# uce/flink-cooccurrence

Hardware: AMD Instinct MI355X
Metric: item-pair co-occurrences counted/sec (node) at 1/2/4/8 GPUs; achieved HBM GB/s (higher is better)
Workload: dtype u32

## Files before the change

flink-cooccurrence_amd/csrc/cooc_sparse.hip:

```cpp
#include "cooc_sparse.h"
#include <algorithm>
#include <cstdio>
#include <string>

namespace cooc {

namespace {

constexpr int kMaxProbe = 64;
constexpr int kSpU = 4;

template <int kWaves>
__device__ inline uint32_t block_excl_scan(uint32_t x, uint32_t *total, uint32_t *s_wtot) {
  const int lane = threadIdx.x & 63, wave = threadIdx.x >> 6;
  const uint32_t inc = wave_incl_scan(x);
  if (lane == 63) s_wtot[wave] = inc;
  __syncthreads();
  uint32_t pre = 0, tot = 0;
#pragma unroll
  for (int w = 0; w < kWaves; w++) {
    const uint32_t v = s_wtot[w];
    pre += w < wave ? v : 0u;
    tot += v;
  }
  __syncthreads();
  *total = uni(tot);
  return pre + inc - x;
}

struct SpShared {
  uint32_t *R;
  uint32_t *L1;
  uint32_t *L1pre;
  int32_t *gb;
  uint32_t *info;
  uint32_t *vst;
  int32_t *qstart;
};

struct SpStatic {
  uint32_t wtot[kSpWaves];
  uint64_t red[kSpWaves];
  int32_t work;
  uint32_t flag;
  int64_t slab_cur, slab_end, row_begin, row_n, pos, copy_from, copy_n;
  int64_t saved_cur, saved_end;
  uint32_t own;
  uint32_t bstart[kSpMaxTiles + 1];
  uint32_t bcur[kSpMaxTiles];
  uint64_t ovf;
  unsigned long long rsum;
#ifdef COOC_SP_STATS
  unsigned long long st[64];
#endif
};

__device__ inline void sp_hash_insert4(uint32_t *keys, uint32_t *cnts, const uint4 &v, uint32_t hshift, uint32_t hmask,
                                       SpStatic &S_) {
  uint32_t k[4] = {v.x + 1u, v.y + 1u, v.z + 1u, v.w + 1u};
  uint32_t h[4];
#pragma unroll
  for (int i = 0; i < 4; i++) h[i] = (k[i] - 1u) * 0x9E3779B1u >> hshift;
#ifdef COOC_SP_STATS
  if (threadIdx.x == 0) S_.st[24] += (k[0] != 0u) + (k[1] != 0u) + (k[2] != 0u) + (k[3] != 0u);
#endif
  for (int p = 0; p < kMaxProbe; p++) {
#ifdef COOC_SP_STATS
    if (threadIdx.x == 0) S_.st[25] += 1;
#endif
    uint32_t cur[4];
#pragma unroll
    for (int i = 0; i < 4; i++) cur[i] = k[i] ? atomicCAS(keys + h[i], 0u, k[i]) : 0u;
    bool left = false;
#pragma unroll
    for (int i = 0; i < 4; i++) {
      if (!k[i]) continue;
      if (cur[i] == 0u || cur[i] == k[i]) {
        atomicAdd(cnts + h[i], 1u);
        k[i] = 0u;
      } else {
        h[i] = (h[i] + 1u) & hmask;
        left = true;
      }
    }
    if (!left) return;
  }
  S_.flag = 1u;
}

constexpr int kWalkDense = 0;
constexpr int kWalkHash = 1;
constexpr int kWalkGather = 2;
struct WalkOp {
  int mode;
  uint32_t hshift, hmask;
  int64_t sbase;
#ifdef COOC_SP_STATS
  bool split;
#endif
};

template <int kOff, int kW>
__device__ inline uint32_t sp_bits(uint32_t w) {
  uint32_t r;
  asm("v_bfe_u32 %0, %1, %2, %3" : "=v"(r) : "v"(w), "n"(kOff), "n"(kW));
  return r;
}

template <class Sh, int kSh>
__device__ inline void sp_dense_add_bit(uint32_t *R, uint32_t w, uint32_t bit) {
  if (Sh::kU16)
    atomicAdd(&R[sp_bits<kSh + 1, kTShift - 1>(w)], bit << (((w >> kSh) & 1u) << 4));
  else
    atomicAdd(&R[sp_bits<kSh, kTShift>(w)], bit);
}

template <class Sh, int kIds, int kMode>
__device__ inline void sp_apply_group(const SpArgs &A, const SpShared &L, SpStatic &S_, const WalkOp &op,
                                      const uint4 &v, uint32_t m) {
  const uint32_t w[4] = {v.x, v.y, v.z, v.w};
  if (kMode == kWalkHash) {
    uint32_t x[kIds];
#pragma unroll
    for (int i = 0; i < 4; i++) {
      if (kIds == 4) {
        x[i] = w[i];
      } else {
        x[2 * i] = w[i] & 0xFFFFu;
        x[2 * i + 1] = w[i] >> 16;
      }
    }
#pragma unroll
    for (int i = 0; i < kIds; i++)
      if (!((m >> i) & 1u)) x[i] = kSink;
#pragma unroll
    for (int h = 0; h < kIds; h += 4)
      sp_hash_insert4(L.R, L.R + Sh::kHashMax, make_uint4(x[h], x[h + 1], x[h + 2], x[h + 3]), op.hshift, op.hmask, S_);
  } else if (kMode == kWalkGather && kIds == 4) {
    uint32_t *scr = reinterpret_cast<uint32_t *>(A.scratch + op.sbase);
#pragma unroll
    for (int i = 0; i < 4; i++) {
      if (!((m >> i) & 1u)) continue;
      const uint32_t t = w[i] >> kTShift;
      const uint32_t slot = atomicAdd(&S_.bcur[t], 1u);
      if (slot < S_.bstart[t + 1] - S_.bstart[t]) scr[S_.bstart[t] + slot] = w[i];
    }
  } else if (kIds == 4) {
#pragma unroll
    for (int i = 0; i < 4; i++) sp_dense_add_bit<Sh, 0>(L.R, w[i], (m >> i) & 1u);
  } else {
#pragma unroll
    for (int i = 0; i < 4; i++) {
      sp_dense_add_bit<Sh, 0>(L.R, w[i], (m >> (2 * i)) & 1u);
      sp_dense_add_bit<Sh, 16>(L.R, w[i], (m >> (2 * i + 1)) & 1u);
    }
  }
// ... 97 lines not shown
      }
#pragma unroll
      for (int k = 0; k < kSpU; k++) v[k] = vn[k];
      m = mn;
    }
  }
  __syncthreads();
  if (kMode == kWalkHash) STAT_ADD(17, STAT_CLOCK() - c_b1);
  return total;
}

template <class Sh>
__device__ inline uint64_t sp_walk(const SpArgs &A, const SpShared &L, SpStatic &S_, int64_t k0, int64_t k1, int t0,
                                   int t1, bool full, bool bucket, const WalkOp &op) {
  uint64_t walked = 0;
  const int tid = threadIdx.x;
  const bool okt = SP_CHECK(A, t0 >= 0 && t1 <= A.T && t0 <= t1);
  const bool has0 = !bucket && (full || t0 == 0);
  const int ta = full ? 1 : max(t0, 1), tz = full ? A.T : t1;
  const bool has1 = bucket || tz > ta;
  if (bucket) {
    k0 = 0;
    k1 = t1 - t0;
  }
  const uint4 *const ar1 = bucket ? A.scratch + op.sbase : A.tarena;
  const int64_t nsrc1 = bucket ? A.scr_cap : A.n_groups;
  const bool rec = !bucket && A.tbc && (full || (t0 == 0 && !has1));
  constexpr uint32_t kNoList = 0xFFFFFFFFu;
  auto list_of = [&](int64_t b) -> uint32_t {
    if (b + tid >= k1 || !okt) return kNoList;
    const uint32_t u = SP_CHECK(A, b + tid < A.n_contrib) ? A.vals[b + tid] & kListMask : 0u;
    return SP_CHECK(A, u < A.n_users) ? u : 0u;
  };
  auto rec_of = [&](uint32_t u) -> int4 { return u != kNoList ? A.tbc[u] : make_int4(0, 0, 0, 0); };
  int4 rn = make_int4(0, 0, 0, 0);
  uint32_t un = kNoList;
  static_assert(Sh::kDb == Sh::kThreads, "a batch: one contribution per thread");
  if (rec && Sh::kAhead) {
    const uint32_t u0 = list_of(k0);
    un = list_of(k0 + Sh::kDb);
    rn = rec_of(u0);
  }
  for (int64_t b0 = k0; b0 < k1; b0 += Sh::kDb) {
    const int nb = int(min<int64_t>(Sh::kDb, k1 - b0));
    uint32_t s0 = 0, e0 = 0, s1 = 0, e1 = 0;
    STAT_ADD(19, op.mode == kWalkHash && !bucket ? 1 : 0);
    if (bucket) {
      if (tid < nb) {
        s1 = S_.bstart[t0 + tid];
        e1 = s1 + S_.bcur[t0 + tid];
      }
    } else if (rec) {
      if (!Sh::kAhead) rn = rec_of(list_of(b0));
      s0 = uint32_t(rn.x);
      e0 = uint32_t(rn.y);
      if (has1) {
        s1 = uint32_t(rn.z);
        e1 = uint32_t(rn.w);
      }
      if (Sh::kAhead) {
        rn = rec_of(un);
        un = list_of(b0 + 2 * Sh::kDb);
      }
    } else if (tid < nb && okt) {
      const uint32_t u = SP_CHECK(A, b0 + tid < A.n_contrib) ? A.vals[b0 + tid] & kListMask : 0u;
      const int32_t *tbu = A.tb + int64_t(SP_CHECK(A, u < A.n_users) ? u : 0u) * (A.T + 2);
      if (has0) {
        s0 = uint32_t(tbu[0]);
        e0 = uint32_t(tbu[A.T + 1]);
      }
      if (has1) {
        s1 = uint32_t(tbu[ta]);
        e1 = uint32_t(tbu[tz]);
      }
    }
    const unsigned long long c_w0 = STAT_CLOCK();
    if (has0) {
      if (op.mode == kWalkHash)
        walked += sp_walk_batch<Sh, 8, kWalkHash>(A, L, S_, A.tarena0, A.n_groups0, nb, s0, e0, op);
      else
        walked += sp_walk_batch<Sh, 8, kWalkDense>(A, L, S_, A.tarena0, A.n_groups0, nb, s0, e0, op);
    }
    const unsigned long long c_w1 = STAT_CLOCK();
    if (has1) {
      if (op.mode == kWalkHash)
        walked += sp_walk_batch<Sh, 4, kWalkHash>(A, L, S_, ar1, nsrc1, nb, s1, e1, op);
      else if (op.mode == kWalkGather)
        walked += sp_walk_batch<Sh, 4, kWalkGather>(A, L, S_, ar1, nsrc1, nb, s1, e1, op);
      else
        walked += sp_walk_batch<Sh, 4, kWalkDense>(A, L, S_, ar1, nsrc1, nb, s1, e1, op);
    }
#ifdef COOC_SP_STATS
    if (op.split) {
      STAT_ADD(56, c_w1 - c_w0);
      STAT_ADD(57, STAT_CLOCK() - c_w1);
    }
#endif
    if (uni(S_.flag)) break;
  }
  return walked;
}

__device__ inline void sp_global_sync() {
  __builtin_amdgcn_s_waitcnt(0);
  __syncthreads();
  __builtin_amdgcn_fence(__ATOMIC_ACQUIRE, "agent");
}

template <class Sh>
__device__ inline int64_t sp_reserve(const SpArgs &A, SpStatic &S_, int64_t n) {
  const int tid = threadIdx.x;
  if (tid == 0) {
    S_.copy_n = 0;
    if (S_.slab_cur + n > S_.slab_end) {
      const int64_t need = S_.row_n + n;
      const int64_t take = max(A.slab, need + need / 2);
      int64_t b = int64_t(atomicAdd(A.bump, (unsigned long long)take));
      if (b + take > A.cap) {
        atomicOr(reinterpret_cast<unsigned long long *>(&A.tot->err), 4ull);
        S_.pos = -1;
      } else {
        S_.copy_from = S_.row_begin;
        S_.copy_n = S_.row_n;
        S_.row_begin = b;
        S_.slab_cur = b + S_.row_n;
        S_.slab_end = b + take;
        S_.pos = S_.slab_cur;
        S_.slab_cur += n;
      }
    } else {
      S_.pos = S_.slab_cur;
      S_.slab_cur += n;
    }
    if (S_.pos >= 0) S_.row_n += n;
  }
  __syncthreads();
  const int64_t cn = uni(S_.copy_n);
  if (cn > 0) {
    sp_global_sync();
    const int64_t from = S_.copy_from, to = S_.row_begin;
    for (int64_t i = tid; i < cn; i += Sh::kThreads) {
      if (SP_CHECK(A, to + i < A.cap && from + i < A.cap && from >= 0)) {
        A.col_out[to + i] = A.col_out[from + i];
        A.cnt_out[to + i] = A.cnt_out[from + i];
      }
    }
  }
  return uni(S_.pos);
}

template <class Sh>
__device__ inline void sp_dense_compact(const SpArgs &A, const SpShared &L, SpStatic &S_, int32_t w, int32_t c0,
                                        uint64_t &rsum, uint32_t *mdst) {
  constexpr int kPer = Sh::kPer, kStep = 64 * kPer, kQ = kPer / 4;
  const int tid = threadIdx.x, lane = tid & 63, wave = tid >> 6;
  const unsigned long long c_d0 = STAT_CLOCK();
  uint32_t *row = L.R;
  if (mdst) {
    const int32_t mh = min(w, A.mirror_hi);
    for (int32_t i = tid; i < mh; i += Sh::kThreads) {
      const uint32_t v = Sh::kU16 ? (row[i >> 1] >> ((i & 1) << 4)) & 0xFFFFu : row[i];
      if (!v) continue;
      const int32_t sl = A.mslot[i];
      if (sl >= 0) mdst[int64_t(sl) * A.sstride] = v;
    }
  }
  const int32_t per = ((w + Sh::kWaves - 1) / Sh::kWaves + kStep - 1) & ~(kStep - 1);
  const int32_t lo = min(w, wave * per), hi = min(w, lo + per);
  const uint4 *row4 = reinterpret_cast<const uint4 *>(row);
  auto load = [&](int32_t b, uint32_t v[kPer]) {
    if (b < hi) {
      const uint4 q = row4[b / kPer];
      const uint32_t ww[4] = {q.x, q.y, q.z, q.w};
#pragma unroll
      for (int k = 0; k < kPer; k++) {
        const uint32_t x = Sh::kU16 ? (ww[k >> 1] >> (16 * (k & 1))) & 0xFFFFu : ww[k & 3];
        v[k] = b + k < hi ? x : 0u;
      }
    } else {
#pragma unroll
      for (int k = 0; k < kPer; k++) v[k] = 0u;
    }
  };
  uint32_t cnt = 0;
  for (int32_t b0 = lo; b0 < hi; b0 += kStep) {
    uint32_t v[kPer];
    load(b0 + kPer * lane, v);
#pragma unroll
    for (int k = 0; k < kPer; k++) cnt += v[k] != 0u;
  }
  for (int o = 32; o > 0; o >>= 1) cnt += __shfl_xor(cnt, o, 64);
  if (lane == 0) S_.wtot[wave] = cnt;
  __syncthreads();
  STAT_ADD(48, STAT_CLOCK() - c_d0);
  uint32_t off = 0, tot = 0;
#pragma unroll
  for (int wv = 0; wv < Sh::kWaves; wv++) {
    const uint32_t x = S_.wtot[wv];
    off += wv < wave ? x : 0u;
    tot += x;
  }
  const bool map = A.hot_col != nullptr && c0 == 0;
  auto colq = [&](int32_t b, uint4 q[kQ]) {
#pragma unroll
    for (int j = 0; j < kQ; j++)
      q[j] = (map && b < hi) ? *reinterpret_cast<const uint4 *>(A.hot_col + b + 4 * j) : make_uint4(0u, 0u, 0u, 0u);
  };
  uint4 q0[kQ], q1[kQ];
  colq(lo + kPer * lane, q0);
  colq(lo + kStep + kPer * lane, q1);
  const int64_t base = sp_reserve<Sh>(A, S_, tot);
  STAT_ADD(49, STAT_CLOCK() - c_d0);
  const uint64_t lt_mask = (lane == 0) ? 0ull : (~0ull >> (64 - lane));
  for (int32_t b0 = lo; b0 < hi; b0 += kStep) {
    const int32_t b = b0 + kPer * lane;
    uint32_t ids[kPer];
#pragma unroll
    for (int j = 0; j < kQ; j++) {
      ids[4 * j] = q0[j].x;
      ids[4 * j + 1] = q0[j].y;
      ids[4 * j + 2] = q0[j].z;
      ids[4 * j + 3] = q0[j].w;
      q0[j] = q1[j];
    }
    colq(b0 + 2 * kStep + kPer * lane, q1);
    uint32_t v[kPer];
    load(b, v);
    uint32_t c = 0;
#pragma unroll
    for (int k = 0; k < kPer; k++) c += v[k] != 0u;
    const uint64_t m0 = __ballot(c & 1u), m1 = __ballot(c & 2u), m2 = __ballot(c & 4u);
    const uint64_t m3 = kPer > 4 ? __ballot(c & 8u) : 0ull;
    const uint32_t pre = uint32_t(__popcll(m0 & lt_mask)) + 2u * uint32_t(__popcll(m1 & lt_mask)) +
                         4u * uint32_t(__popcll(m2 & lt_mask)) + 8u * uint32_t(__popcll(m3 & lt_mask));
#pragma unroll
    for (int k = 0; k < kPer; k++) rsum += v[k];
    if (c) {
      int64_t pos = base + off + pre;
#pragma unroll
      for (int k = 0; k < kPer; k++) {
        if (!v[k]) continue;
        if (base >= 0) {
          if (SP_CHECK(A, pos >= 0 && pos < A.cap)) {
            A.col_out[pos] = map ? int32_t(ids[k]) : c0 + b + k - (A.hot_col ? kTW : 0);
            A.cnt_out[pos] = v[k];
          }
        }
        pos++;
      }
      reinterpret_cast<uint4 *>(row)[b / kPer] = make_uint4(0u, 0u, 0u, 0u);
    }
    off += uint32_t(__popcll(m0)) + 2u * uint32_t(__popcll(m1)) + 4u * uint32_t(__popcll(m2)) +
           8u * uint32_t(__popcll(m3));
  }
  STAT_ADD(50, STAT_CLOCK() - c_d0);
  __syncthreads();
  STAT_ADD(51, STAT_CLOCK() - c_d0);
}

template <class Sh>
__device__ inline void sp_hash_compact(const SpArgs &A, const SpShared &L, SpStatic &S_, int32_t H, int32_t c0,
                                       int32_t c1, uint64_t &rsum, uint32_t *mdst) {
  const int tid = threadIdx.x;
  const unsigned long long c_h0 = STAT_CLOCK();
  const uint32_t mhi = mdst ? uint32_t(A.mirror_hi) : 0u;
  uint32_t *keys = L.R, *cnts = L.R + Sh::kHashMax;
  const int per = H / Sh::kThreads;
  const int32_t nL1 = (c1 - c0 + 1023) >> 10;
  uint32_t ek[Sh::kHashMax / Sh::kThreads], ec[Sh::kHashMax / Sh::kThreads], er[Sh::kHashMax / Sh::kThreads];
  (void)per;
#pragma unroll
  for (int q = 0; q < Sh::kHashMax / (4 * Sh::kThreads); q++) {
    const int j = 4 * (tid + q * Sh::kThreads);
    uint4 k4 = make_uint4(0u, 0u, 0u, 0u), v4 = k4;
    if (j < H) {
      k4 = *reinterpret_cast<const uint4 *>(keys + j);
      v4 = *reinterpret_cast<const uint4 *>(cnts + j);
      *reinterpret_cast<uint4 *>(keys + j) = make_uint4(0u, 0u, 0u, 0u);
      *reinterpret_cast<uint4 *>(cnts + j) = make_uint4(0u, 0u, 0u, 0u);
    }
    const uint32_t kk[4] = {k4.x, k4.y, k4.z, k4.w}, vv[4] = {v4.x, v4.y, v4.z, v4.w};
#pragma unroll
    for (int u = 0; u < 4; u++) {
      const int i = 4 * q + u;
      ek[i] = ~0u;
      ec[i] = 0u;
      er[i] = 0u;
      if (kk[u] && vv[u]) {
        const uint32_t col = kk[u] - 1u - uint32_t(c0);
        ek[i] = col;
        ec[i] = vv[u];
        rsum += vv[u];
        if (col < mhi) {
          const int32_t sl = A.mslot[col];
          if (sl >= 0) mdst[int64_t(sl) * A.sstride] = vv[u];
        }
        if (Sh::kRank && !A.any_order) atomicOr(&L.L1[col >> 10], 1u << ((col >> 5) & 31u));
      }
    }
  }
  __syncthreads();
  STAT_ADD(46, STAT_CLOCK() - c_h0);
  if (!Sh::kRank || A.any_order) {
    uint32_t cnt = 0;
#pragma unroll
    for (int i = 0; i < Sh::kHashMax / Sh::kThreads; i++) cnt += ek[i] != ~0u;
    uint32_t ne;
    uint32_t q = block_excl_scan<Sh::kWaves>(cnt, &ne, S_.wtot);
    const unsigned long long c_a1 = STAT_CLOCK();
    STAT_ADD(20, c_a1 - c_h0);
    const int64_t base = sp_reserve<Sh>(A, S_, ne);
    const unsigned long long c_a2 = STAT_CLOCK();
    STAT_ADD(21, c_a2 - c_a1);
    if (base >= 0 && ne <= uint32_t(Sh::kWStage)) {
      uint32_t *sc = keys + Sh::kWStage, *sn = cnts + Sh::kWStage;
#pragma unroll
      for (int i = 0; i < Sh::kHashMax / Sh::kThreads; i++) {
        if (ek[i] == ~0u) continue;
        sc[q] = uint32_t(sp_col(A, uint32_t(c0) + ek[i]));
        sn[q] = ec[i];
        q++;
      }
      __syncthreads();
      const uint32_t head = min(ne, uint32_t((4 - (base & 3)) & 3));
      const uint32_t body = (ne - head) >> 2;
      for (uint32_t j = tid; j < head; j += Sh::kThreads) {
        A.col_out[base + j] = int32_t(sc[j]);
        A.cnt_out[base + j] = sn[j];
      }
      int4 *co4 = reinterpret_cast<int4 *>(A.col_out + base + head);
      uint4 *cn4 = reinterpret_cast<uint4 *>(A.cnt_out + base + head);
      for (uint32_t j = tid; j < body; j += Sh::kThreads) {
        const uint32_t r = head + 4 * j;
        co4[j] = make_int4(int32_t(sc[r]), int32_t(sc[r + 1]), int32_t(sc[r + 2]), int32_t(sc[r + 3]));
        cn4[j] = make_uint4(sn[r], sn[r + 1], sn[r + 2], sn[r + 3]);
      }
      for (uint32_t r = head + 4 * body + tid; r < ne; r += Sh::kThreads) {
        A.col_out[base + r] = int32_t(sc[r]);
        A.cnt_out[base + r] = sn[r];
      }
      __syncthreads();
      for (uint32_t r = tid; r < ne; r += Sh::kThreads) {
        sc[r] = 0u;
        sn[r] = 0u;
      }
    } else if (base >= 0) {
#pragma unroll
      for (int i = 0; i < Sh::kHashMax / Sh::kThreads; i++) {
        if (ek[i] == ~0u) continue;
        if (SP_CHECK(A, base + q < A.cap)) {
          A.col_out[base + q] = sp_col(A, uint32_t(c0) + ek[i]);
          A.cnt_out[base + q] = ec[i];
        }
        q++;
      }
    }
    __syncthreads();
    STAT_ADD(22, STAT_CLOCK() - c_a2);
    STAT_ADD(23, ne);
    return;
  }
  if constexpr (Sh::kRank) {
  uint32_t nblk;
  {
    static_assert(Sh::kL1Words % Sh::kThreads == 0, "L1 words per thread");
    constexpr int kW = Sh::kL1Words / Sh::kThreads;
    uint32_t pc[kW], x = 0;
#pragma unroll
    for (int i = 0; i < kW; i++) {
      pc[i] = kW * tid + i < nL1 ? uint32_t(__popc(L.L1[kW * tid + i])) : 0u;
      x += pc[i];
    }
    const uint32_t p = block_excl_scan<Sh::kWaves>(x, &nblk, S_.wtot);
    uint32_t run = p;
#pragma unroll
    for (int i = 0; i < kW; i++) {
      if (kW * tid + i < nL1) L.L1pre[kW * tid + i] = run;
      run += pc[i];
    }
  }
  __syncthreads();
#pragma unroll
  for (int i = 0; i < Sh::kHashMax / Sh::kThreads; i++) {
    if (ek[i] == ~0u) continue;
    const uint32_t col = ek[i], wd = col >> 10, bit = (col >> 5) & 31u;
    const uint32_t r = L.L1pre[wd] + uint32_t(__popc(L.L1[wd] & ((1u << bit) - 1u)));
    er[i] = r;
    atomicOr(&keys[r], 1u << (col & 31u));
  }
  __syncthreads();
  STAT_ADD(47, STAT_CLOCK() - c_h0);
  const uint32_t pb = (nblk + Sh::kThreads - 1) / Sh::kThreads;
  const uint32_t r0 = min(nblk, uint32_t(tid) * pb), r1 = min(nblk, r0 + pb);
  uint32_t local = 0;
  for (uint32_t r = r0; r < r1; r++) local += uint32_t(__popc(keys[r]));
  uint32_t ne;
  uint32_t run = block_excl_scan<Sh::kWaves>(local, &ne, S_.wtot);
  for (uint32_t r = r0; r < r1; r++) {
    cnts[r] = run;
    run += uint32_t(__popc(keys[r]));
  }
  const unsigned long long c_h1 = STAT_CLOCK();
  STAT_ADD(20, c_h1 - c_h0);
  const int64_t base = sp_reserve<Sh>(A, S_, ne);
  const unsigned long long c_h2 = STAT_CLOCK();
  STAT_ADD(21, c_h2 - c_h1);
  if (base >= 0 && ne <= uint32_t(Sh::kWStage)) {
// ... 209 lines not shown
        __syncthreads();
        STAT_ADD(26, STAT_CLOCK() - c_walked);
      } else if (dense) {
        if (tid == 0 && ra >= c0 && ra < c1) {
          const uint32_t o = uint32_t(ra - c0);
          if (Sh::kU16)
            L.R[o >> 1] -= self << ((o & 1u) << 4);
          else
            L.R[o] -= self;
        }
        __syncthreads();
        sp_dense_compact<Sh>(A, L, S_, c1 - c0, c0, rsum, c0 == 0 ? mdst : nullptr);
        STAT_ADD(2, STAT_CLOCK() - c_walked);
      } else {
        if (tid == 0 && ra >= c0 && ra < c1) {
          uint32_t h = (uint32_t(ra) * 0x9E3779B1u) >> op.hshift;
          for (int p = 0; p < H; p++) {
            if (L.R[h] == uint32_t(ra) + 1u) {
              L.R[Sh::kHashMax + h] -= self;
              break;
            }
            h = (h + 1u) & op.hmask;
          }
        }
        __syncthreads();
        sp_hash_compact<Sh>(A, L, S_, H, c0, c1, rsum, c0 == 0 ? mdst : nullptr);
        STAT_ADD(3, STAT_CLOCK() - c_walked);
#ifdef COOC_SP_STATS
        STAT_ADD(30 + 6 * hcls, STAT_CLOCK() - c_walked);
        STAT_ADD(32 + 6 * hcls, uni(S_.row_n));
#endif
        STAT_ADD(14, H);
      }
      t = t1;
      H = 0;
    }
    STAT_ADD(split ? 12 : 11, 1);
    if (deferred) {
      STAT_ADD(8, 1);
      rsum = 0;
      if (tid == 0) {
        A.deferred[atomicAdd(reinterpret_cast<unsigned long long *>(&A.tot->n_deferred), 1ull)] = a;
        if (!S_.own) S_.slab_cur = S_.row_begin;
        S_.row_n = 0;
      }
    }
    if (!split) {
      for (int o = 32; o > 0; o >>= 1) rsum += __shfl_xor(rsum, o, 64);
      if ((tid & 63) == 0 && rsum) atomicAdd(&S_.rsum, (unsigned long long)rsum);
    }
    rsum = 0;
    if (!split && tid == 0) {
      A.row_base[a] = S_.row_n ? S_.row_begin : 0;
      A.row_nnz[a] = int32_t(S_.row_n);
      if (S_.own) {
        S_.slab_cur = S_.saved_cur;
        S_.slab_end = S_.saved_end;
      }
    }
    if (tid == 0) S_.work = next;
    __syncthreads();
    if (!split && !deferred && tid == 0 && S_.rsum != (unsigned long long)rs_expect) {
      atomicOr(reinterpret_cast<unsigned long long *>(&A.tot->err), 2ull);
      A.tot->bad_row = a;
    }
  }
#ifdef COOC_SP_STATS
  if (tid == 0) {
    S_.st[13] = STAT_CLOCK() - t_start;
    for (int k = 0; k < 64; k++) atomicAdd(A.stats + k, S_.st[k]);
  }
#endif
}

constexpr int kFinThreads = 1024, kFinWaves = kFinThreads / 64, kFinU = 4;
__global__ __launch_bounds__(kFinThreads) void k_sp_split_finalize(const int32_t *__restrict__ split_row,
                                                                    const uint32_t *__restrict__ staging, int64_t stride,
                                                                    int32_t M, const int64_t *__restrict__ row_ptr,
                                                                    const int64_t *__restrict__ rowsum,
                                                                    int32_t *__restrict__ col_out,
                                                                    uint32_t *__restrict__ cnt_out,
                                                                    unsigned long long *__restrict__ bump, int64_t cap,
                                                                    int64_t *__restrict__ row_base,
                                                                    int32_t *__restrict__ row_nnz,
                                                                    PlanTotals *__restrict__ tot,
                                                                    const int64_t *__restrict__ spre,
                                                                    const int32_t *__restrict__ hot_col,
                                                                    const int32_t *__restrict__ pos_of) {
  __shared__ uint32_t s_w[kFinWaves];
  __shared__ uint64_t s_red[kFinWaves];
  __shared__ int64_t s_base;
  const int tid = threadIdx.x, lane = tid & 63, wave = tid >> 6;
  const int32_t s = blockIdx.x;
  const int32_t a = split_row[s];
  const int32_t ra = relabel_pos(pos_of, uint32_t(a));
  const uint32_t self = uint32_t(spre ? spre[row_ptr[a + 1]] - spre[row_ptr[a]] : row_ptr[a + 1] - row_ptr[a]);
  const uint32_t *row = staging + int64_t(s) * stride;
  constexpr int32_t kStep = 64 * 4 * kFinU;
  const int32_t per = ((M + kFinWaves - 1) / kFinWaves + kStep - 1) / kStep * kStep;
  const int32_t lo = min(M, wave * per), hi = min(M, lo + per);
  auto load = [&](int32_t b, uint32_t v[4]) {
    if (b + 3 < hi) {
      const uint4 q = *reinterpret_cast<const uint4 *>(row + b);
      v[0] = q.x;
      v[1] = q.y;
      v[2] = q.z;
      v[3] = q.w;
    } else {
      for (int k = 0; k < 4; k++) v[k] = b + k < hi ? row[b + k] : 0u;
    }
    for (int k = 0; k < 4; k++)
      if (b + k == ra) v[k] -= self;
  };
  uint32_t cnt = 0;
  uint64_t sum = 0;
  for (int32_t b0 = lo; b0 < hi; b0 += kStep) {
    uint32_t v[kFinU][4];
#pragma unroll
    for (int u = 0; u < kFinU; u++) load(b0 + (u * 64 + lane) * 4, v[u]);
#pragma unroll
    for (int u = 0; u < kFinU; u++)
#pragma unroll
      for (int k = 0; k < 4; k++) {
        cnt += v[u][k] != 0u;
        sum += v[u][k];
      }
  }
  for (int o = 32; o > 0; o >>= 1) cnt += __shfl_xor(cnt, o, 64);
  if (lane == 0) s_w[wave] = cnt;
  for (int o = 32; o > 0; o >>= 1) sum += __shfl_xor(sum, o, 64);
  if (lane == 0) s_red[wave] = sum;
  __syncthreads();
  uint32_t off = 0, tot_n = 0;
  uint64_t total_sum = 0;
  for (int w = 0; w < kFinWaves; w++) {
    off += w < wave ? s_w[w] : 0u;
    tot_n += s_w[w];
    total_sum += s_red[w];
  }
  if (tid == 0) {
    int64_t b = int64_t(atomicAdd(bump, (unsigned long long)tot_n));
    if (b + int64_t(tot_n) > cap) {
      atomicOr(reinterpret_cast<unsigned long long *>(&tot->err), 4ull);
      b = -1;
    }
    s_base = b;
    row_base[a] = b < 0 ? 0 : b;
    row_nnz[a] = int32_t(tot_n);
    if (total_sum != uint64_t(rowsum[a])) atomicOr(reinterpret_cast<unsigned long long *>(&tot->err), 2ull);
  }
  __syncthreads();
  const int64_t base = s_base;
  if (base < 0) return;
  const uint64_t lt_mask = (lane == 0) ? 0ull : (~0ull >> (64 - lane));
  for (int32_t b0 = lo; b0 < hi; b0 += kStep) {
    uint32_t v[kFinU][4];
#pragma unroll
    for (int u = 0; u < kFinU; u++) load(b0 + (u * 64 + lane) * 4, v[u]);
#pragma unroll
    for (int u = 0; u < kFinU; u++) {
      const int32_t b = b0 + (u * 64 + lane) * 4;
      const uint32_t c = (v[u][0] != 0u) + (v[u][1] != 0u) + (v[u][2] != 0u) + (v[u][3] != 0u);
      const uint64_t m0 = __ballot(c & 1u), m1 = __ballot(c & 2u), m2 = __ballot(c & 4u);
      int64_t pos = base + off + uint32_t(__popcll(m0 & lt_mask)) + 2u * uint32_t(__popcll(m1 & lt_mask)) +
                    4u * uint32_t(__popcll(m2 & lt_mask));
#pragma unroll
      for (int k = 0; k < 4; k++)
        if (v[u][k]) {
          col_out[pos] = relabel_col(hot_col, uint32_t(b + k));
          cnt_out[pos] = v[u][k];
          pos++;
        }
      off += uint32_t(__popcll(m0)) + 2u * uint32_t(__popcll(m1)) + 4u * uint32_t(__popcll(m2));
    }
  }
}

__global__ void k_sp_nnz_total(const int32_t *__restrict__ row_nnz, int32_t M, PlanTotals *__restrict__ tot) {
  __shared__ uint64_t s[4];
  uint64_t v = 0;
  for (int32_t a = blockIdx.x * 256 + threadIdx.x; a < M; a += gridDim.x * 256) v += uint64_t(row_nnz[a]);
  for (int o = 32; o > 0; o >>= 1) v += __shfl_xor(v, o, 64);
  if ((threadIdx.x & 63) == 0) s[threadIdx.x >> 6] = v;
  __syncthreads();
  if (threadIdx.x == 0) {
    const uint64_t t = s[0] + s[1] + s[2] + s[3];
    if (t) atomicAdd(reinterpret_cast<unsigned long long *>(&tot->nnz_total), (unsigned long long)t);
  }
}

__global__ void k_sp_reset_run(PlanTotals *__restrict__ tot, int32_t *__restrict__ qctr,
                               unsigned long long *__restrict__ bump) {
  tot->err &= ~int64_t(6);
  tot->nnz_total = 0;
  tot->n_deferred = 0;
  tot->tiny_ctr = 0;
  tot->small_ctr = 0;
  qctr[0] = qctr[1] = 0;
  bump[0] = 0;
}


int64_t sp_scratch(int64_t max_tail, int64_t g, int32_t T, DevBuf &buf) {
  if (max_tail <= 0) return 0;
  const int64_t sc = std::min<int64_t>(kScrGroups, (max_tail + max_tail / 4 + 64 * T + 4096) / 4 + 1);
  const size_t need = sizeof(uint4) * size_t(g) * size_t(sc);
  size_t f0 = 0, t0 = 0;
  if (hipMemGetInfo(&f0, &t0) != hipSuccess) return 0;
  if (need > buf.cap && (need > (f0 + buf.cap) / 4 || !buf.reserve(need).ok())) return 0;
  return sc;
}

#ifdef COOC_SP_STATS
unsigned long long *sp_stats_buf() {
  static unsigned long long *d_stats = nullptr;
  if (!d_stats) (void)hipMalloc(reinterpret_cast<void **>(&d_stats), 128 * 8);
  return d_stats;
}
#endif

}

Status Counter::sparse_sizes(SparseRun &R) {
  const int32_t M = M_, T = R.T;
  const PlanTotals &t = R.tot;
  const int64_t n_split = t.n_split;
  R.sstride = (int64_t(R.Mc) + 3) & ~int64_t(3);
  if (n_split > 0) {
    const size_t need = sizeof(uint32_t) * size_t(n_split) * size_t(R.sstride);
    COOC_TRY(staging_.reserve(need));
  }
  const int64_t n_tiny = t.n_tiny, n_small = t.n_small, n_mid = t.n_mid;
  const int64_t n_big = t.n_chunks - n_tiny - n_small - n_mid;
  COOC_HIP_TRY(hipFuncSetAttribute(reinterpret_cast<const void *>(k_sp_main<SpBig>),
                                   hipFuncAttributeMaxDynamicSharedMemorySize, SpBig::kLds));
  COOC_HIP_TRY(hipFuncSetAttribute(reinterpret_cast<const void *>(k_sp_main<SpMid>),
                                   hipFuncAttributeMaxDynamicSharedMemorySize, SpMid::kLds));
  COOC_HIP_TRY(hipFuncSetAttribute(reinterpret_cast<const void *>(k_sp_main<SpMidAny>),
                                   hipFuncAttributeMaxDynamicSharedMemorySize, SpMidAny::kLds));
  R.mid_any = any_order_ && !R.win && !mid4_off_;
  int per_cu = 1, per_cu_mid = 1;
  COOC_HIP_TRY(hipOccupancyMaxActiveBlocksPerMultiprocessor(&per_cu, k_sp_main<SpBig>, SpBig::kThreads, SpBig::kLds));
  if (R.mid_any)
    COOC_HIP_TRY(hipOccupancyMaxActiveBlocksPerMultiprocessor(&per_cu_mid, k_sp_main<SpMidAny>, SpMidAny::kThreads,
                                                              SpMidAny::kLds));
  else
    COOC_HIP_TRY(hipOccupancyMaxActiveBlocksPerMultiprocessor(&per_cu_mid, k_sp_main<SpMid>, SpMid::kThreads, SpMid::kLds));
  R.grid = std::min<int64_t>(std::max<int64_t>(n_big, 1), int64_t(n_cu_) * std::max(1, per_cu));
  R.grid_mid = std::min<int64_t>(std::max<int64_t>(n_mid, 1), int64_t(n_cu_) * std::max(1, per_cu_mid));
  R.scr_cap = sp_scratch(R.mirror ? t.max_tail : std::max(t.max_tail, t.max_tail_split), R.grid, T, sp_scr_);
  R.scr_cap_mid = n_mid > 0 ? sp_scratch(t.max_tail_mid, R.grid_mid, T, sp_scr_mid_) : 0;
  R.n_gather = t.n_gather_rows + (R.mirror ? 0 : t.n_split_work);
  size_t free_b = 0, total_b = 0;
  COOC_HIP_TRY(hipMemGetInfo(&free_b, &total_b));
  R.slab = std::max<int64_t>(int64_t(1) << 16, std::min<int64_t>(int64_t(1) << 22, t.est_nnz / (8 * R.grid)));
  R.grid_tiny = std::min<int64_t>((n_tiny + kTinyWaves - 1) / kTinyWaves, int64_t(n_cu_) * 8);
  R.grid_small = std::min<int64_t>(n_small, int64_t(n_cu_) * 4);
  R.slack = 2 * R.grid * R.slab + (n_mid ? 2 * R.grid_mid * R.slab : 0) + M +
            (n_tiny ? R.grid_tiny * kTinyWaves * kTinySlab : 0) + (n_small ? R.grid_small * kSmallSlab : 0) +
            2 * int64_t(n_cu_) * kSmallSlab;
  R.cap = std::min<int64_t>(t.cap_total + R.slack, t.est_nnz + t.est_nnz / 4 + R.slack);
  const int64_t budget = int64_t((free_b + col_.cap + cnt_.cap) / 10 * 8 / 8);
  R.cap = std::max<int64_t>(1, std::min(R.cap, budget));
  dense_mode_ = false;
  last_rows_ = M;
  COOC_TRY(bump_.reserve(sizeof(uint64_t) * 2));
  SpArgs &A = R.proto;
  A.queue = sp_queue_.as<SpWork>();
  A.tot = tot_.as<PlanTotals>();
  A.qctr = queue_.as<int32_t>();
  A.vals = vals_out_.as<uint32_t>();
  A.tb = sp_tb_.as<int32_t>();
  A.tbc = tbc_off_ ? nullptr : sp_tbc_.as<int4>();
  A.tarena = sp_arena_.as<uint4>();
  A.tarena0 = sp_arena0_.as<uint4>();
  A.epre = epre_.as<int64_t>();
  A.gmass = sp_est_.as<float>() + T * kEstK;
  A.split_slot = split_slot_.as<int32_t>();
  A.bump = bump_.as<unsigned long long>();
  A.slab = R.slab;
  A.row_base = row_base_.as<int64_t>();
  A.row_nnz = row_nnz_.as<int32_t>();
  A.M = R.Mc;
  A.T = T;
  A.n_contrib = R.n_c;
  A.n_users = R.U;
  A.n_groups = R.n_groups1;
  A.n_groups0 = R.n_groups0;
  A.scratch = R.scr_cap ? sp_scr_.as<uint4>() : nullptr;
  A.scr_cap = (R.scr_cap && R.n_gather) ? R.scr_cap : 0;
  A.rowsum = rowsum_.as<int64_t>();
  A.spre = R.spre;
  COOC_TRY(sp_defer_.reserve(sizeof(int32_t) * size_t(M)));
  A.deferred = sp_defer_.as<int32_t>();
  A.sort_all = sort_rows_ ? 1 : 0;
  A.any_order = (any_order_ && !R.win) ? 1 : 0;
  A.hot_col = R.hot_col;
  A.pos_of = R.pos_of;
  A.mslot = R.mirror ? sp_mslot_.as<int32_t>() : nullptr;
  A.mirror_hi = R.mirror ? int32_t(std::min<int64_t>(t.split_rank_hi, kTW)) : 0;
  return Status::Ok();
}

Status Counter::sparse_attempt(SparseRun &R, int64_t *err, int64_t *n_def) {
  hipStream_t s = R.s;
  const PlanTotals &t = R.tot;
  const int64_t n_split = t.n_split, n_tiny = t.n_tiny, n_small = t.n_small, n_mid = t.n_mid;
  const int64_t n_big = t.n_chunks - n_tiny - n_small - n_mid;
  PlanTotals *tot = tot_.as<PlanTotals>();
  COOC_TRY(col_.reserve(sizeof(int32_t) * size_t(R.cap + 1)));
  COOC_TRY(cnt_.reserve(sizeof(uint32_t) * size_t(R.cap + 1)));
  if (n_split > 0)
    COOC_HIP_TRY(hipMemsetAsync(staging_.p, 0, sizeof(uint32_t) * size_t(n_split) * size_t(R.sstride), s));
  k_sp_reset_run<<<1, 1, 0, s>>>(tot, R.proto.qctr, bump_.as<unsigned long long>());
  SpArgs A = R.proto;
#ifdef COOC_SP_STATS
  A.stats = sp_stats_buf();
  (void)hipMemsetAsync(A.stats, 0, 128 * 8, s);
#endif
  A.staging = staging_.as<uint32_t>();
  A.sstride = R.sstride;
  A.col_out = col_.as<int32_t>();
  A.cnt_out = cnt_.as<uint32_t>();
  A.cap = R.cap;
  if (R.timer && R.timer->enabled) COOC_HIP_TRY(hipEventRecord(R.timer->acc_begin, s));
  A.q_begin = 0;
// ... 164 lines not shown
```

Measured before the change: 356.0 billion.

## Switch dense compaction to lane-strided element ownership with mbcnt prefix and coalesced stores

The dense row compaction and the final-row emit now assign consecutive elements to consecutive lanes (strided by 64) instead of giving each lane a contiguous run of kPer elements. Output positions come from one ballot plus mbcnt per element rather than multi-bit ballots and popcounts, so neighbouring lanes write neighbouring output slots and the stores coalesce better. The hot-column id prefetch is rebuilt to match the new ownership, with a waitcnt and a compile-time split between mapped and unmapped paths. In exchange the code issues more ballots and narrower loads per element, and the changed per-lane bounds handling could introduce correctness problems.

```diff
diff --git a/flink-cooccurrence_amd/csrc/cooc_sparse.hip b/flink-cooccurrence_amd/csrc/cooc_sparse.hip
--- a/flink-cooccurrence_amd/csrc/cooc_sparse.hip
+++ b/flink-cooccurrence_amd/csrc/cooc_sparse.hip
@@ -2,6 +2,7 @@
 #include <algorithm>
 #include <cstdio>
 #include <string>
+#include <type_traits>
 
 namespace cooc {
 
@@ -405,7 +406,7 @@
 template <class Sh>
 __device__ inline void sp_dense_compact(const SpArgs &A, const SpShared &L, SpStatic &S_, int32_t w, int32_t c0,
                                         uint64_t &rsum, uint32_t *mdst) {
-  constexpr int kPer = Sh::kPer, kStep = 64 * kPer, kQ = kPer / 4;
+  constexpr int kPer = Sh::kPer, kStep = 64 * kPer;
   const int tid = threadIdx.x, lane = tid & 63, wave = tid >> 6;
   const unsigned long long c_d0 = STAT_CLOCK();
   uint32_t *row = L.R;
@@ -454,58 +455,77 @@
     tot += x;
   }
   const bool map = A.hot_col != nullptr && c0 == 0;
-  auto colq = [&](int32_t b, uint4 q[kQ]) {
-#pragma unroll
-    for (int j = 0; j < kQ; j++)
-      q[j] = (map && b < hi) ? *reinterpret_cast<const uint4 *>(A.hot_col + b + 4 * j) : make_uint4(0u, 0u, 0u, 0u);
+  constexpr int kW = Sh::kU16 ? 2 : 1, kSub = kPer / kW;
+  const int32_t cshift = c0 - (A.hot_col ? kTW : 0);
+  uint32_t nxt[kSub][kW];
+  auto colq = [&](int32_t b0, bool on) {
+#pragma unroll
+    for (int k = 0; k < kSub; k++) {
+      const int32_t b = b0 + kW * (64 * k + lane);
+      if (Sh::kU16) {
+        const uint2 t = (on && b < hi) ? *reinterpret_cast<const uint2 *>(A.hot_col + b) : make_uint2(0u, 0u);
+        nxt[k][0] = t.x;
+        nxt[k][kW - 1] = t.y;
+      } else {
+        nxt[k][0] = (on && b < hi) ? uint32_t(A.hot_col[b]) : 0u;
+      }
+    }
   };
-  uint4 q0[kQ], q1[kQ];
-  colq(lo + kPer * lane, q0);
-  colq(lo + kStep + kPer * lane, q1);
+  colq(lo, map);
   const int64_t base = sp_reserve<Sh>(A, S_, tot);
   STAT_ADD(49, STAT_CLOCK() - c_d0);
-  const uint64_t lt_mask = (lane == 0) ? 0ull : (~0ull >> (64 - lane));
-  for (int32_t b0 = lo; b0 < hi; b0 += kStep) {
-    const int32_t b = b0 + kPer * lane;
-    uint32_t ids[kPer];
-#pragma unroll
-    for (int j = 0; j < kQ; j++) {
-      ids[4 * j] = q0[j].x;
-      ids[4 * j + 1] = q0[j].y;
-      ids[4 * j + 2] = q0[j].z;
-      ids[4 * j + 3] = q0[j].w;
-      q0[j] = q1[j];
-    }
-    colq(b0 + 2 * kStep + kPer * lane, q1);
-    uint32_t v[kPer];
-    load(b, v);
-    uint32_t c = 0;
-#pragma unroll
-    for (int k = 0; k < kPer; k++) c += v[k] != 0u;
-    const uint64_t m0 = __ballot(c & 1u), m1 = __ballot(c & 2u), m2 = __ballot(c & 4u);
-    const uint64_t m3 = kPer > 4 ? __ballot(c & 8u) : 0ull;
-    const uint32_t pre = uint32_t(__popcll(m0 & lt_mask)) + 2u * uint32_t(__popcll(m1 & lt_mask)) +
-                         4u * uint32_t(__popcll(m2 & lt_mask)) + 8u * uint32_t(__popcll(m3 & lt_mask));
-#pragma unroll
-    for (int k = 0; k < kPer; k++) rsum += v[k];
-    if (c) {
-      int64_t pos = base + off + pre;
-#pragma unroll
-      for (int k = 0; k < kPer; k++) {
-        if (!v[k]) continue;
-        if (base >= 0) {
-          if (SP_CHECK(A, pos >= 0 && pos < A.cap)) {
-            A.col_out[pos] = map ? int32_t(ids[k]) : c0 + b + k - (A.hot_col ? kTW : 0);
-            A.cnt_out[pos] = v[k];
+  off = uni(off);
+  auto sweep = [&](auto mapped) {
+    constexpr bool kMap = decltype(mapped)::value;
+    for (int32_t b0 = lo; b0 < hi; b0 += kStep) {
+      uint32_t word[kSub], ids[kSub][kW] = {};
+#pragma unroll
+      for (int k = 0; k < kSub; k++) {
+        const int32_t b = b0 + kW * (64 * k + lane);
+        word[k] = b < hi ? row[b / kW] : 0u;
+      }
+      if constexpr (kMap) {
+#pragma unroll
+        for (int k = 0; k < kSub; k++)
+#pragma unroll
+          for (int j = 0; j < kW; j++) ids[k][j] = nxt[k][j];
+        __builtin_amdgcn_s_waitcnt(0x0F70);
+        colq(b0 + kStep, true);
+      }
+#pragma unroll
+      for (int k = 0; k < kSub; k++) {
+        const int32_t b = b0 + kW * (64 * k + lane);
+        const uint32_t x0 = Sh::kU16 ? word[k] & 0xFFFFu : word[k];
+        const uint32_t x1 = (Sh::kU16 && b + 1 < hi) ? word[k] >> 16 : 0u;
+        const uint64_t m0 = __ballot(x0 != 0u), m1 = Sh::kU16 ? __ballot(x1 != 0u) : 0ull;
+        uint32_t pre = __builtin_amdgcn_mbcnt_hi(uint32_t(m0 >> 32), __builtin_amdgcn_mbcnt_lo(uint32_t(m0), 0u));
+        if (Sh::kU16) pre = __builtin_amdgcn_mbcnt_hi(uint32_t(m1 >> 32), __builtin_amdgcn_mbcnt_lo(uint32_t(m1), pre));
+        rsum += x0 + x1;
+        if (word[k]) {
+          const int64_t pos = base + off;
+          int32_t *const cp = A.col_out + pos;
+          uint32_t *const np = A.cnt_out + pos;
+          const uint32_t pre1 = pre + (x0 != 0u);
+          if (base >= 0) {
+            if (x0 && SP_CHECK(A, pos >= 0 && pos + pre < A.cap)) {
+              cp[pre] = kMap ? int32_t(ids[k][0]) : cshift + b;
+              np[pre] = x0;
+            }
+            if (Sh::kU16 && x1 && SP_CHECK(A, pos >= 0 && pos + pre1 < A.cap)) {
+              cp[pre1] = kMap ? int32_t(ids[k][kW - 1]) : cshift + b + 1;
+              np[pre1] = x1;
+            }
           }
+          row[b / kW] = 0u;
         }
-        pos++;
-      }
-      reinterpret_cast<uint4 *>(row)[b / kPer] = make_uint4(0u, 0u, 0u, 0u);
-    }
-    off += uint32_t(__popcll(m0)) + 2u * uint32_t(__popcll(m1)) + 4u * uint32_t(__popcll(m2)) +
-           8u * uint32_t(__popcll(m3));
-  }
+        off += uint32_t(__popcll(m0)) + uint32_t(__popcll(m1));
+      }
+    }
+  };
+  if (map)
+    sweep(std::true_type{});
+  else
+    sweep(std::false_type{});
   STAT_ADD(50, STAT_CLOCK() - c_d0);
   __syncthreads();
   STAT_ADD(51, STAT_CLOCK() - c_d0);
@@ -1021,26 +1041,25 @@
   __syncthreads();
   const int64_t base = s_base;
   if (base < 0) return;
-  const uint64_t lt_mask = (lane == 0) ? 0ull : (~0ull >> (64 - lane));
+  constexpr int kSub = kStep / 64;
   for (int32_t b0 = lo; b0 < hi; b0 += kStep) {
-    uint32_t v[kFinU][4];
-#pragma unroll
-    for (int u = 0; u < kFinU; u++) load(b0 + (u * 64 + lane) * 4, v[u]);
-#pragma unroll
-    for (int u = 0; u < kFinU; u++) {
-      const int32_t b = b0 + (u * 64 + lane) * 4;
-      const uint32_t c = (v[u][0] != 0u) + (v[u][1] != 0u) + (v[u][2] != 0u) + (v[u][3] != 0u);
-      const uint64_t m0 = __ballot(c & 1u), m1 = __ballot(c & 2u), m2 = __ballot(c & 4u);
-      int64_t pos = base + off + uint32_t(__popcll(m0 & lt_mask)) + 2u * uint32_t(__popcll(m1 & lt_mask)) +
-                    4u * uint32_t(__popcll(m2 & lt_mask));
-#pragma unroll
-      for (int k = 0; k < 4; k++)
-        if (v[u][k]) {
-          col_out[pos] = relabel_col(hot_col, uint32_t(b + k));
-          cnt_out[pos] = v[u][k];
-          pos++;
-        }
-      off += uint32_t(__popcll(m0)) + 2u * uint32_t(__popcll(m1)) + 4u * uint32_t(__popcll(m2));
+    uint32_t v[kSub];
+#pragma unroll
+    for (int j = 0; j < kSub; j++) {
+      const int32_t b = b0 + 64 * j + lane;
+      v[j] = b < hi ? row[b] : 0u;
+      if (b == ra) v[j] -= self;
+    }
+#pragma unroll
+    for (int j = 0; j < kSub; j++) {
+      const int32_t b = b0 + 64 * j + lane;
+      const uint64_t m = __ballot(v[j] != 0u);
+      if (v[j]) {
+        const uint32_t pre = __builtin_amdgcn_mbcnt_hi(uint32_t(m >> 32), __builtin_amdgcn_mbcnt_lo(uint32_t(m), 0u));
+        (col_out + (base + off))[pre] = relabel_col(hot_col, uint32_t(b));
+        (cnt_out + (base + off))[pre] = v[j];
+      }
+      off += uint32_t(__popcll(m));
     }
   }
 }
```

After: 365.8 billion (median of 6 runs). +2.8%, better.
